# miha-stopar/Plonky3-mobile

Hardware: AMD Instinct MI355X
Metric: fib_air proofs/sec (higher is better)
Workload: dtype u32 (BabyBear Montgomery, 31-bit modular)

## Files before the change

include/p3hip.h:

```cpp
#ifndef P3HIP_H
#define P3HIP_H
#include <stddef.h>
#include <stdint.h>

#ifdef __cplusplus
extern "C" {
#endif

#define P3HIP_OK 0
#define P3HIP_ERR_BAD_ARG (-1)
#define P3HIP_ERR_HIP (-2)
#define P3HIP_ERR_BACKEND (-3)
#define P3HIP_ERR_INTERNAL (-4)

#define P3HIP_BACKEND_CPU 0
#define P3HIP_BACKEND_VULKAN 1
#define P3HIP_BACKEND_METAL 2
#define P3HIP_BACKEND_WEBGPU 3
#define P3HIP_BACKEND_HIP 4

int p3hip_set_backend(const char *name);
int p3hip_get_backend(void);
int p3hip_is_available(char *msg, size_t cap);
const char *p3hip_take_last_error(void);
// ... 10 lines not shown
int p3hip_coset_dft_batch_bb31(const uint32_t *in, uint32_t *out, size_t height, size_t width,
                               uint32_t shift_monty);
int p3hip_coset_lde_batch_bb31(const uint32_t *in, uint32_t *out, size_t height, size_t width,
                               unsigned added_bits, uint32_t shift_monty, int bit_reversed_out);
const char *p3hip_last_timing_line(void);
int p3hip_dft_batch_bb31_dev(const uint32_t *d_in, uint32_t *d_out, size_t height, size_t width, void *stream);
int p3hip_idft_batch_bb31_dev(const uint32_t *d_in, uint32_t *d_out, size_t height, size_t width, void *stream);
int p3hip_coset_dft_batch_bb31_dev(const uint32_t *d_in, uint32_t *d_out, size_t height, size_t width,
                                   uint32_t shift_monty, void *stream);
int p3hip_coset_lde_batch_bb31_dev(const uint32_t *d_in, uint32_t *d_out, size_t height, size_t width,
                                   unsigned added_bits, uint32_t shift_monty, int bit_reversed_out,
                                   void *stream);
int p3hip_coset_lde_from_coeffs_bb31_dev(const uint32_t *d_coeffs, uint32_t *d_out, size_t height, size_t width,
                                         unsigned added_bits, uint32_t shift_monty, void *stream);
int p3hip_dft_plan_bb31(size_t height, size_t width, uint32_t *stages_per_pass, size_t cap, size_t *n_passes);
int p3hip_bit_reverse_rows_dev(const uint32_t *d_in, uint32_t *d_out, size_t height, size_t width, void *stream);

int p3hip_fib_trace_dev(uint64_t a, uint64_t b, size_t n, uint32_t *d_out, void *stream);

int p3hip_poseidon2_permute_dev(uint32_t *d_states, size_t n, void *stream);
int p3hip_poseidon2_permute(uint32_t *states, size_t n);
int p3hip_poseidon2_permute_variant_dev(uint32_t *d_states, size_t n, int variant, void *stream);
int p3hip_poseidon2_f64_probe_dev(const double *d_in, uint32_t *d_out, size_t n, int mode, void *stream);

typedef struct p3hip_tree p3hip_tree_t;
int p3hip_mmcs_commit_dev(const uint32_t *const *d_mats, const size_t *heights, const size_t *widths,
                          size_t n_mats, uint32_t root_out[8], p3hip_tree_t **tree_out, void *stream);
int p3hip_mmcs_commit_async_dev(const uint32_t *const *d_mats, const size_t *heights, const size_t *widths,
                                size_t n_mats, p3hip_tree_t **tree_out, void *stream);
int p3hip_mmcs_root(const p3hip_tree_t *tree, uint32_t root_out[8], void *stream);
size_t p3hip_mmcs_log_max_height(const p3hip_tree_t *tree);
size_t p3hip_mmcs_num_layers(const p3hip_tree_t *tree);
const uint32_t *p3hip_mmcs_layer_dev(const p3hip_tree_t *tree, size_t layer, size_t *len_out);
int p3hip_mmcs_open_batch(const p3hip_tree_t *tree, size_t index, uint32_t *rows_out, uint32_t *path_out,
                          void *stream);
void p3hip_mmcs_free(p3hip_tree_t *tree);
int p3hip_mmcs_commit(const uint32_t *const *mats, const size_t *heights, const size_t *widths,
                      size_t n_mats, uint32_t root_out[8], p3hip_tree_t **tree_out);

#define P3HIP_HASH_POSEIDON2 0
#define P3HIP_HASH_KECCAK 1
int p3hip_mmcs_commit_hash_dev(int hash, const uint32_t *const *d_mats, const size_t *heights, const size_t *widths,
                               size_t n_mats, uint32_t root_out[8], p3hip_tree_t **tree_out, void *stream);
int p3hip_mmcs_commit_hash(int hash, const uint32_t *const *mats, const size_t *heights, const size_t *widths,
                           size_t n_mats, uint32_t root_out[8], p3hip_tree_t **tree_out);
size_t p3hip_mmcs_layer_words(size_t max_height);
// ... 91 lines not shown
```

plonky3-mobile_amd/_lib.py:

```python
import ctypes as C
import os
import subprocess

_HERE = os.path.dirname(os.path.abspath(__file__))
LIB_PATH = os.environ.get("P3HIP_LIB") or os.path.join(_HERE, "libp3hip.so")
ROOT = os.path.dirname(_HERE)

u32p = C.POINTER(C.c_uint32)
_SIGS = {
    "p3hip_set_backend": (C.c_int, [C.c_char_p]),
    "p3hip_get_backend": (C.c_int, []),
    "p3hip_is_available": (C.c_int, [C.c_char_p, C.c_size_t]),
    "p3hip_take_last_error": (C.c_char_p, []),
    "p3hip_malloc": (C.c_int, [C.POINTER(C.c_void_p), C.c_size_t]),
    "p3hip_free": (C.c_int, [C.c_void_p]),
    "p3hip_upload": (C.c_int, [C.c_void_p, C.c_void_p, C.c_size_t]),
    "p3hip_download": (C.c_int, [C.c_void_p, C.c_void_p, C.c_size_t]),
    "p3hip_sync": (C.c_int, [C.c_void_p]),
    "p3hip_last_timing_line": (C.c_char_p, []),
    "p3hip_release_thread_context": (None, []),
    "p3hip_dft_batch_bb31": (C.c_int, [C.c_void_p, C.c_void_p, C.c_size_t, C.c_size_t]),
    "p3hip_idft_batch_bb31": (C.c_int, [C.c_void_p, C.c_void_p, C.c_size_t, C.c_size_t]),
    "p3hip_coset_dft_batch_bb31": (C.c_int, [C.c_void_p, C.c_void_p, C.c_size_t, C.c_size_t, C.c_uint32]),
    "p3hip_coset_lde_batch_bb31": (C.c_int, [C.c_void_p, C.c_void_p, C.c_size_t, C.c_size_t, C.c_uint,
                                             C.c_uint32, C.c_int]),
    "p3hip_dft_batch_bb31_dev": (C.c_int, [C.c_void_p, C.c_void_p, C.c_size_t, C.c_size_t, C.c_void_p]),
    "p3hip_idft_batch_bb31_dev": (C.c_int, [C.c_void_p, C.c_void_p, C.c_size_t, C.c_size_t, C.c_void_p]),
    "p3hip_coset_dft_batch_bb31_dev": (C.c_int, [C.c_void_p, C.c_void_p, C.c_size_t, C.c_size_t, C.c_uint32,
                                                 C.c_void_p]),
    "p3hip_coset_lde_batch_bb31_dev": (C.c_int, [C.c_void_p, C.c_void_p, C.c_size_t, C.c_size_t, C.c_uint,
                                                 C.c_uint32, C.c_int, C.c_void_p]),
    "p3hip_coset_lde_from_coeffs_bb31_dev": (C.c_int, [C.c_void_p, C.c_void_p, C.c_size_t, C.c_size_t, C.c_uint, C.c_uint32,
                                                       C.c_void_p]),
    "p3hip_bit_reverse_rows_dev": (C.c_int, [C.c_void_p, C.c_void_p, C.c_size_t, C.c_size_t, C.c_void_p]),
    "p3hip_dft_plan_bb31": (C.c_int, [C.c_size_t, C.c_size_t, C.POINTER(C.c_uint32), C.c_size_t, C.POINTER(C.c_size_t)]),
    "p3hip_fib_trace_dev": (C.c_int, [C.c_uint64, C.c_uint64, C.c_size_t, C.c_void_p, C.c_void_p]),
    "p3hip_poseidon2_permute_dev": (C.c_int, [C.c_void_p, C.c_size_t, C.c_void_p]),
    "p3hip_poseidon2_permute": (C.c_int, [C.c_void_p, C.c_size_t]),
    "p3hip_poseidon2_permute_variant_dev": (C.c_int, [C.c_void_p, C.c_size_t, C.c_int, C.c_void_p]),
    "p3hip_poseidon2_f64_probe_dev": (C.c_int, [C.c_void_p, C.c_void_p, C.c_size_t, C.c_int, C.c_void_p]),
    "p3hip_mmcs_commit_dev": (C.c_int, [C.POINTER(C.c_void_p), C.POINTER(C.c_size_t), C.POINTER(C.c_size_t),
                                        C.c_size_t, C.c_void_p, C.POINTER(C.c_void_p), C.c_void_p]),
    "p3hip_mmcs_commit_async_dev": (C.c_int, [C.POINTER(C.c_void_p), C.POINTER(C.c_size_t),
                                              C.POINTER(C.c_size_t), C.c_size_t, C.POINTER(C.c_void_p),
                                              C.c_void_p]),
    "p3hip_mmcs_commit_hash_dev": (C.c_int, [C.c_int, C.POINTER(C.c_void_p), C.POINTER(C.c_size_t), C.POINTER(C.c_size_t),
                                             C.c_size_t, C.c_void_p, C.POINTER(C.c_void_p), C.c_void_p]),
    "p3hip_mmcs_commit_hash": (C.c_int, [C.c_int, C.POINTER(C.c_void_p), C.POINTER(C.c_size_t), C.POINTER(C.c_size_t),
                                         C.c_size_t, C.c_void_p, C.POINTER(C.c_void_p)]),
    "p3hip_mmcs_layer_words": (C.c_size_t, [C.c_size_t]),
    "p3hip_mmcs_commit_into_dev": (C.c_int, [C.c_int, C.POINTER(C.c_void_p), C.POINTER(C.c_size_t), C.POINTER(C.c_size_t),
                                             C.c_size_t, C.c_void_p, C.POINTER(C.c_void_p), C.c_void_p]),
    "p3hip_keccak_f_dev": (C.c_int, [C.c_void_p, C.c_size_t, C.c_void_p]),
    "p3hip_mmcs_root": (C.c_int, [C.c_void_p, C.c_void_p, C.c_void_p]),
    "p3hip_mmcs_log_max_height": (C.c_size_t, [C.c_void_p]),
    "p3hip_mmcs_num_layers": (C.c_size_t, [C.c_void_p]),
    "p3hip_mmcs_layer_dev": (C.c_void_p, [C.c_void_p, C.c_size_t, C.POINTER(C.c_size_t)]),
    "p3hip_mmcs_open_batch": (C.c_int, [C.c_void_p, C.c_size_t, C.c_void_p, C.c_void_p, C.c_void_p]),
    "p3hip_mmcs_free": (None, [C.c_void_p]),
    "p3hip_set_thread_profile": (C.c_int, [C.c_int]),
    "p3hip_get_thread_profile": (C.c_int, []),
    "p3hip_fib_prover_create_profile": (C.c_int, [C.c_int, C.c_int, C.c_int, C.c_uint64, C.c_uint, C.c_void_p, C.c_void_p, C.c_int,
                                                  C.POINTER(C.c_void_p)]),
# ... 126 lines not shown
```

plonky3-mobile_amd/csrc/c_api.hip:

```cpp
#include "../../include/p3hip.h"

#include <atomic>
#include <chrono>
#include <condition_variable>
#include <mutex>
#include <deque>
#include <thread>
#include <cctype>
#include <cstdio>
#include <cstring>

#include "bb31.hip.h"
#include "common.h"
#include "mmcs.h"
#include "prover.h"
#include "rng.h"

namespace p3 {
bool take_error(std::string* out);
}
using namespace p3;

static std::atomic<uint8_t> g_backend{P3HIP_BACKEND_HIP};

// ... 269 lines not shown
        P3_HIP(hipMemcpy(states, cx->ws(stream, 2).ptr, n * 64, hipMemcpyDeviceToHost));
        return OK;
    });
}

int p3hip_poseidon2_permute_variant_dev(uint32_t* d_states, size_t n, int variant, void* stream) {
    return guarded([&]() -> int {
        if (n && !d_states) return fail(ERR_BAD_ARG, "null state pointer");
        if (variant != 0 && variant != 1) return fail(ERR_BAD_ARG, "poseidon2 variant: 0 = int32, 1 = fp64");
        Context* cx;
        int rc = get_context(&cx);
        if (rc) return rc;
        return poseidon2_permute_states_variant((hipStream_t)stream, d_states, n, variant);
    });
}
int p3hip_poseidon2_f64_probe_dev(const double* d_in, uint32_t* d_out, size_t n, int mode, void* stream) {
    return guarded([&]() -> int {
        if (n && (!d_in || !d_out)) return fail(ERR_BAD_ARG, "null pointer");
        if (mode < 0 || mode > 2) return fail(ERR_BAD_ARG, "probe mode: 0 = permutation, 1 = internal rounds, 2 = reduce");
        Context* cx;
        int rc = get_context(&cx);
        if (rc) return rc;
        return poseidon2_f64_probe((hipStream_t)stream, d_in, d_out, n, mode);
    });
}

}
struct p3hip_tree {
    Tree* t;
};
extern "C" {

static int commit_async_kind(int kind, const uint32_t* const* d_mats, const size_t* heights, const size_t* widths,
                             size_t n_mats, p3hip_tree_t** tree_out, void* stream) {
    return guarded([&]() -> int {
        if (!tree_out) return fail(ERR_BAD_ARG, "mmcs_commit: null tree_out");
        Context* cx;
        int rc = get_context(&cx);
        if (rc) return rc;
        Tree* t = nullptr;
        rc = mmcs_commit((hipStream_t)stream, d_mats, heights, widths, n_mats, &t, nullptr, nullptr, kind, nullptr, cx->profile);
        if (rc) return rc;
        *tree_out = new p3hip_tree{t};
        return OK;
    });
}
// ... 705 lines not shown
```

plonky3-mobile_amd/csrc/mmcs.h:

```cpp
#pragma once
#include <memory>
#include <cstring>
#include "common.h"

namespace p3 {

enum HashKind : int { HASH_POSEIDON2 = 0, HASH_KECCAK = 1 };

struct Tree {
    int kind = HASH_POSEIDON2;
    std::vector<const uint32_t*> mats;
    std::vector<size_t> heights, widths, strides;
    std::vector<void*> owned;
    uint32_t* layers = nullptr;
    bool root_copied = false;
    bool owns_layers = true;
    std::vector<size_t> layer_off, layer_len;
    uint32_t log_max_height = 0;
    uint32_t* staging = nullptr;
    size_t staging_words = 0;
    ~Tree();
};

int mmcs_commit(hipStream_t stream, const uint32_t* const* d_mats, const size_t* heights, const size_t* widths,
                size_t n_mats, Tree** out, uint32_t* ext_layers = nullptr, uint32_t* root_copy = nullptr,
                int kind = HASH_POSEIDON2, const size_t* strides = nullptr, int profile = PROFILE_LATENCY);
inline size_t mmcs_layer_words(uint64_t max_height) { return (size_t)(2 * max_height - 1) * 8; }
int mmcs_root(hipStream_t stream, const Tree& t, uint32_t root_out[8]);
int mmcs_open(hipStream_t stream, const Tree& t, uint64_t index, uint32_t* rows_out, uint32_t* path_out);
int poseidon2_permute_states(hipStream_t stream, uint32_t* d_states, uint64_t n);
int poseidon2_f64_probe(hipStream_t stream, const double* d_in, uint32_t* d_out, uint64_t n, int mode);
int poseidon2_permute_states_variant(hipStream_t stream, uint32_t* d_states, uint64_t n, int variant);
int keccak_f_states(hipStream_t stream, uint64_t* d_states, uint64_t n);

}
```

plonky3-mobile_amd/csrc/mmcs.hip:

```cpp
#include <algorithm>

#include "common.h"
#include "mmcs.h"
#include "poseidon2.hip.h"
#include "poseidon2_coop.hip.h"
#include "poseidon2_f64.hip.h"
#include "poseidon2_q4.hip.h"
#include "keccak.hip.h"

namespace p3 {

constexpr int MAX_CLASS_MATS = 16;

struct RowSet {
    const uint32_t* ptr[MAX_CLASS_MATS];
    uint32_t width[MAX_CLASS_MATS];
    uint32_t stride[MAX_CLASS_MATS];
    uint32_t count;
    uint32_t total;
};

__device__ __forceinline__ void load_digest(const uint32_t* p, uint32_t* out8) {
    const uint4* q = reinterpret_cast<const uint4*>(p);
    uint4 a = q[0], b = q[1];
// ... 94 lines not shown
    if (gridDim.x <= 512u) P3_LATENCY_BOUND_KERNEL();
    uint64_t r = (uint64_t)blockIdx.x * blockDim.x + threadIdx.x;
    if (r >= n_rows) return;
    double s[16];
#pragma unroll
    for (int i = 0; i < 16; i++) s[i] = 0.0;
    const uint32_t* row = mat + r * width;
    for (uint32_t k = 0; k < width; k += 8) {
#pragma unroll
        for (int i = 0; i < 8; i++)
            if (k + i < width) s[i] = p2f::load_elem(row[k + i]);
        p2f::permute(s);
        if (k + 8 < width) {
#pragma unroll
            for (int i = 0; i < 16; i++) s[i] = p2f::reduce(s[i]);
        }
    }
    uint32_t d[8];
    const p2f::MagicRegs smk = p2f::magic_regs();
#pragma unroll
    for (int i = 0; i < 8; i++) d[i] = p2f::store_elem(s[i], smk);
    store_digest(digests + r * 8, d);
}
__global__ void __launch_bounds__(256) compress_layer_q4_kernel(const uint32_t* prev, uint32_t* next, uint64_t n_out, uint32_t prio) {
    if (prio) P3_LATENCY_BOUND_KERNEL();
    const uint32_t q = threadIdx.x & 3u;
    const uint64_t i = ((uint64_t)blockIdx.x * blockDim.x + threadIdx.x) >> 2;
    const bool act = i < n_out;
    const p2q::LaneConsts lc = p2q::lane_consts(q);
    double s[4] = {0.0, 0.0, 0.0, 0.0};
    if (act) {
        const uint4 w = *reinterpret_cast<const uint4*>(prev + i * 16 + 4 * q);
        s[0] = p2f::load_elem(w.x); s[1] = p2f::load_elem(w.y); s[2] = p2f::load_elem(w.z); s[3] = p2f::load_elem(w.w);
    }
    p2q::permute(s, lc, q == 0);
    if (act && q < 2) {
        const p2f::MagicRegs smk = p2f::magic_regs();
        *reinterpret_cast<uint4*>(next + i * 8 + 4 * q) =
            make_uint4(p2f::store_elem(s[0], smk), p2f::store_elem(s[1], smk), p2f::store_elem(s[2], smk), p2f::store_elem(s[3], smk));
    }
}
__global__ void __launch_bounds__(256) leaf_hash_q4_kernel(const uint32_t* mat, uint32_t width, uint64_t n_rows, uint32_t* digests, uint32_t prio) {
    if (prio) P3_LATENCY_BOUND_KERNEL();
    const uint32_t q = threadIdx.x & 3u;
    const uint64_t r = ((uint64_t)blockIdx.x * blockDim.x + threadIdx.x) >> 2;
    const bool act = r < n_rows;
// ... 56 lines not shown
            }
        }
    }
    if (r >= n_rows) return;
    uint32_t d[8];
    const p2f::MagicRegs smk = p2f::magic_regs();
#pragma unroll
    for (int i = 0; i < 8; i++) d[i] = p2f::store_elem(s[i], smk);
    store_digest(digests + r * 8, d);
}
__global__ void __launch_bounds__(256) leaf_hash_f64_rowset_kernel(RowSet rs, uint64_t n_rows, uint32_t* digests) {
    if (gridDim.x <= 512u) P3_LATENCY_BOUND_KERNEL();
    uint64_t r = (uint64_t)blockIdx.x * blockDim.x + threadIdx.x;
    if (r >= n_rows) return;
    double s[16];
#pragma unroll
    for (int i = 0; i < 16; i++) s[i] = 0.0;
    uint32_t m = 0, off = 0;
    for (uint32_t k = 0; k < rs.total; k += 8) {
#pragma unroll
        for (int i = 0; i < 8; i++) {
            if (k + i < rs.total) {
                while (off >= rs.width[m]) { m++; off = 0; }
                s[i] = p2f::load_elem(rs.ptr[m][r * rs.stride[m] + off]);
                off++;
            }
        }
        p2f::permute(s);
        if (k + 8 < rs.total) {
#pragma unroll
            for (int i = 0; i < 16; i++) s[i] = p2f::reduce(s[i]);
        }
    }
    uint32_t d[8];
    const p2f::MagicRegs smk = p2f::magic_regs();
#pragma unroll
    for (int i = 0; i < 8; i++) d[i] = p2f::store_elem(s[i], smk);
    store_digest(digests + r * 8, d);
}
__global__ void __launch_bounds__(256) compress_layer_f64_kernel(const uint32_t* prev, uint32_t* next, uint64_t n_out) {
    if (gridDim.x <= 512u) P3_LATENCY_BOUND_KERNEL();
    uint64_t i = (uint64_t)blockIdx.x * blockDim.x + threadIdx.x;
    if (i >= n_out) return;
    uint32_t w[16];
    load_digest(prev + i * 16, w);
    load_digest(prev + i * 16 + 8, w + 8);
    double s[16];
#pragma unroll
    for (int k = 0; k < 16; k++) s[k] = p2f::load_elem(w[k]);
    p2f::permute(s);
    uint32_t d[8];
    const p2f::MagicRegs smk = p2f::magic_regs();
#pragma unroll
    for (int k = 0; k < 8; k++) d[k] = p2f::store_elem(s[k], smk);
    store_digest(next + i * 8, d);
}

__global__ void __launch_bounds__(256) compress_coop_kernel(const uint32_t* prev, uint32_t* next, uint32_t n_out) {
    P3_LATENCY_BOUND_KERNEL();
    const uint32_t lane16 = threadIdx.x & 15;
    const p2c::LaneConst lc = p2c::lane_constants(lane16);
    uint32_t i = (blockIdx.x * blockDim.x + threadIdx.x) >> 4;
    bool act = i < n_out;
    uint32_t v = act ? prev[(size_t)i * 16 + lane16] : 0u;
    v = p2c::permute(v, lc);
    if (act && lane16 < 8) next[(size_t)i * 8 + lane16] = v;
}
__global__ void __launch_bounds__(256) leaf_coop_kernel(const uint32_t* mat, uint32_t width, uint32_t n_rows, uint32_t* digests) {
    P3_LATENCY_BOUND_KERNEL();
    const uint32_t lane16 = threadIdx.x & 15;
    const p2c::LaneConst lc = p2c::lane_constants(lane16);
    uint32_t r = (blockIdx.x * blockDim.x + threadIdx.x) >> 4;
    bool act = r < n_rows;
// ... 62 lines not shown
#pragma unroll
    for (int k = 0; k < 4; k++)
        q[k] = make_uint4(p2f::store_elem(s[4 * k]), p2f::store_elem(s[4 * k + 1]), p2f::store_elem(s[4 * k + 2]), p2f::store_elem(s[4 * k + 3]));
}

__global__ void poseidon2_f64_probe_kernel(const double* in, uint32_t* out, uint64_t n, int mode) {
    uint64_t i = (uint64_t)blockIdx.x * blockDim.x + threadIdx.x;
    if (i >= n) return;
    double s[16];
#pragma unroll
    for (int k = 0; k < 16; k++) s[k] = in[i * 16 + k];
    if (mode == 0) p2f::permute(s);
    else if (mode == 1) p2f::internal_rounds(s, p2f::magic_regs());
    else {
#pragma unroll
        for (int k = 0; k < 16; k++) s[k] = p2f::reduce(s[k]);
    }
#pragma unroll
    for (int k = 0; k < 16; k++) out[i * 16 + k] = p2f::store_elem(s[k]);
}
int poseidon2_f64_probe(hipStream_t stream, const double* d_in, uint32_t* d_out, uint64_t n, int mode) {
    if (!n) return OK;
    hipLaunchKernelGGL(poseidon2_f64_probe_kernel, dim3((uint32_t)((n + 255) / 256)), dim3(256), 0, stream, d_in, d_out, n, mode);
    P3_HIP(hipGetLastError());
    return OK;
}
int poseidon2_permute_states_variant(hipStream_t stream, uint32_t* d_states, uint64_t n, int variant) {
    if (!n) return OK;
    if (variant == 1) hipLaunchKernelGGL(poseidon2_permute_f64_kernel, dim3((uint32_t)((n + 255) / 256)), dim3(256), 0, stream, d_states, n);
    else hipLaunchKernelGGL(poseidon2_permute_kernel, dim3((uint32_t)((n + 255) / 256)), dim3(256), 0, stream, d_states, n);
    P3_HIP(hipGetLastError());
    return OK;
}

int poseidon2_permute_states(hipStream_t stream, uint32_t* d_states, uint64_t n) {
    return poseidon2_permute_states_variant(stream, d_states, n, 1);
}

__device__ __forceinline__ uint32_t rowset_elem(const RowSet& rs, uint64_t r, uint32_t k, uint32_t& m, uint32_t& base) {
    while (k - base >= rs.width[m]) { base += rs.width[m]; m++; }
    return rs.ptr[m][r * rs.stride[m] + (k - base)];
}
__device__ __forceinline__ void keccak_sponge_row(const RowSet& rs, uint64_t r, uint64_t (&st)[25]) {
#pragma unroll
    for (int i = 0; i < 25; i++) st[i] = 0;
    const uint32_t n = rs.total, n64 = (n + 1) / 2;
// ... 367 lines not shown
                if (t->layer_len[l + levels - 1] == 1) t->root_copied = root_copy != nullptr;
                l += levels - 1;
                continue;
            }
            hipLaunchKernelGGL(keccak_compress_kernel, dim3((uint32_t)((len + 255) / 256)), dim3(256), 0, stream,
                               t->layers + t->layer_off[l - 1], t->layers + t->layer_off[l], len, rs, rs.count > 0 ? 1u : 0u);
            P3_HIP(hipGetLastError());
        }
        *out = t.release();
        return OK;
    }
    {
        RowSet rs = make_rowset(*t, maxh);
        const bool dense1 = rs.count == 1 && rs.stride[0] == rs.width[0];
        if (dense1 && maxh < COOP_MAX && maxh * 16 <= 0x7fffffffull) {
            hipLaunchKernelGGL(leaf_coop_kernel, dim3((uint32_t)((maxh * 16 + 255) / 256)), dim3(256), 0, stream, rs.ptr[0],
                               rs.width[0], (uint32_t)maxh, t->layers);
        } else if (dense1 && maxh <= Q4_MAX && rs.width[0] <= 64 && (reinterpret_cast<uintptr_t>(t->layers) & 15u) == 0) {
            hipLaunchKernelGGL(leaf_hash_q4_kernel, dim3((uint32_t)((maxh * 4 + 255) / 256)), dim3(256), 0, stream, rs.ptr[0], rs.width[0], maxh,
                               t->layers, Q4_PRIO);
        } else if (dense1 && rs.width[0] >= 64) {
            hipLaunchKernelGGL(leaf_hash_f64_wide_kernel, dim3((uint32_t)((maxh + 255) / 256)), dim3(256), 0, stream, rs.ptr[0],
                               rs.width[0], maxh, t->layers);
        } else if (dense1) {
            hipLaunchKernelGGL(leaf_hash_f64_kernel, dim3((uint32_t)((maxh + 255) / 256)), dim3(256), 0, stream, rs.ptr[0],
                               rs.width[0], maxh, t->layers);
        } else if ((maxh >= COOP_MAX || (rs.count == 1 && !dense1))) {
            hipLaunchKernelGGL(leaf_hash_f64_rowset_kernel, dim3((uint32_t)((maxh + 255) / 256)), dim3(256), 0, stream, rs, maxh, t->layers);
        } else {
            hipLaunchKernelGGL(leaf_hash_kernel, dim3((uint32_t)((maxh + 255) / 256)), dim3(256), 0, stream, rs, maxh, t->layers);
        }
        P3_HIP(hipGetLastError());
    }
    for (size_t l = 1; l < t->layer_len.size();) {
        uint64_t len = t->layer_len[l];
        RowSet rs = make_rowset(*t, len);
        bool inject = rs.count > 0;
        if (!inject && len < COOP_MAX) {
            uint32_t levels = 0;
            while (levels < COOP_CHUNK_LOG && l + levels < t->layer_len.size() && !has_height(*t, t->layer_len[l + levels])) levels++;
            uint64_t n_in = t->layer_len[l - 1];
            uint32_t chunk = (uint32_t)std::min<uint64_t>(n_in, 1ull << COOP_CHUNK_LOG);
            while ((1u << levels) > chunk) levels--;
            uint32_t blocks = (uint32_t)(n_in / chunk);
            uint32_t threads = std::max<uint32_t>(64, chunk * 8);
            bool makes_root = t->layer_len[l + levels - 1] == 1;
// ... 59 lines not shown
```

plonky3-mobile_amd/csrc/poseidon2_f64.hip.h:

```cpp
#pragma once
#include "poseidon2.hip.h"

namespace p2f {

constexpr double PD = 2013265921.0;
constexpr double PINV = 1.0 / 2013265921.0;

__device__ __forceinline__ double mulmod(double a, double b) {
    double h = a * b;
    double l = __fma_rn(a, b, -h);
    double q = __builtin_rint(h * PINV);
    double r = __fma_rn(-q, PD, h);
    return r + l;
}
constexpr double PM1 = 2013265920.0;
__device__ __forceinline__ double mulmod_p(double a, double b, double aP) {
    double q = __builtin_rint(b * aP);
    double t = __fma_rn(a, b, -(q * PM1));
    return t - q;
}
__device__ __forceinline__ double reduce(double x) {
    return __fma_rn(-__builtin_rint(x * PINV), PD, x);
}
__device__ __forceinline__ double add_scaled_pow2(double tot, double x, double inv) {
// ... 84 lines not shown
        s[8] = __fma_rn(s[8], -4.0, tot);
        s[9] = add_scaled_pow2(tot, s[9], i256);
        s[10] = add_scaled_pow2(tot, s[10], i4);
        s[11] = add_scaled_pow2(tot, s[11], i8);
        s[12] = __fma_rn(s[12], -k15, tot);
        s[13] = add_scaled_pow2(tot, s[13], -i256);
        s[14] = add_scaled_pow2(tot, s[14], -i16);
        s[15] = __fma_rn(s[15], k15, tot);
    };
    auto fold_integer_lanes = [&]() {
        s[1] = reduce(s[1]); s[2] = reduce(s[2]); s[4] = reduce(s[4]); s[5] = reduce(s[5]);
        s[7] = reduce(s[7]); s[8] = reduce(s[8]); s[12] = reduce(s[12]); s[15] = reduce(s[15]);
    };
    _Pragma("clang loop unroll(disable)")
    for (int blk = 0; blk < 3; blk++) {
        _Pragma("clang loop unroll(disable)")
        for (int r = 0; r < 4; r++) internal_round(4 * blk + r);
        fold_integer_lanes();
    }
    internal_round(12);
    fold_integer_lanes();
}

__device__ __forceinline__ void permute(double (&s)[16]) {
    const MagicRegs mk = magic_regs();
    const double npm1 = d_c.neg_pm1, pinv = d_c.pinv;
    external_linear(s);
    _Pragma("clang loop unroll(disable)")
    for (int r = 0; r < 4; r++) {
#pragma unroll
        for (int i = 0; i < 16; i++) s[i] = sbox7(s[i] + d_c.ext[r][i], mk, npm1, pinv);
        external_linear(s);
    }
    internal_rounds(s, mk);
    _Pragma("clang loop unroll(disable)")
    for (int r = 4; r < 8; r++) {
#pragma unroll
        for (int i = 0; i < 16; i++) s[i] = sbox7(s[i] + d_c.ext[r][i], mk, npm1, pinv);
        external_linear(s);
    }
}

__device__ __forceinline__ double load_elem(uint32_t monty) { return (double)bb::from_monty(monty); }
constexpr double R_MOD_P = 268435454.0;
constexpr double R_MOD_P_OVER_P = 268435454.0 / 2013265921.0;
__device__ __forceinline__ uint32_t store_elem(double v, const MagicRegs& k) {
    const double r = mulmod_m(R_MOD_P, v, R_MOD_P_OVER_P, k, d_c.neg_pm1);
    const uint32_t w = (uint32_t)(int32_t)r;
    return min(w, w + bb::P);
}
__device__ __forceinline__ uint32_t store_elem(double v) { return store_elem(v, magic_regs()); }

}
```

plonky3-mobile_amd/csrc/prover.hip:

```cpp
#include <chrono>
#include <deque>
#include <memory>
#include <cstring>

#include "bb31.hip.h"
#include "challenger.h"
#include "common.h"
#include "keccak.hip.h"
#include "mmcs.h"
#include "poseidon2.hip.h"
#include "poseidon2_f64.hip.h"
#include "prover.h"
#include "rng.h"
#include "rng_dev.hip.h"
#include "transcript.hip.h"

namespace p3 {

using bb::Ext;

__device__ __forceinline__ uint32_t tl(const TwoLevelTable& t, uint32_t e) {
    return bb::mul(t.lo[e & ((1u << t.T) - 1u)], t.hi[e >> t.T]);
}
__device__ __forceinline__ uint32_t brev(uint32_t v, uint32_t bits) { return bits ? (__brev(v) >> (32 - bits)) : 0u; }
// ... 43 lines not shown
};
__global__ void __launch_bounds__(256) fib_quotient_kernel(QuotArgs a) {
    uint32_t i = blockIdx.x * blockDim.x + threadIdx.x;
    if (i >= a.n) return;
    const DevState* __restrict__ ds = a.ds;
    uint2 loc = a.lde[brev(i, a.log_n)];
    uint2 nxt = a.lde[brev((i + 1) & (a.n - 1), a.log_n)];
    uint2 s = a.sel[i];
    uint32_t x = bb::mul(a.gen, tl(a.roots, i));
    uint32_t trans = bb::sub(x, a.ginv);
    uint32_t c0 = bb::mul(s.x, bb::sub(loc.x, ds->pis[0]));
    uint32_t c1 = bb::mul(s.x, bb::sub(loc.y, ds->pis[1]));
    uint32_t c2 = bb::mul(trans, bb::sub(loc.y, nxt.x));
    uint32_t c3 = bb::mul(trans, bb::sub(bb::add(loc.x, loc.y), nxt.y));
    uint32_t c4 = bb::mul(s.y, bb::sub(loc.y, ds->pis[2]));
    Ext acc;
#pragma unroll
    for (int k = 0; k < 4; k++)
        acc.c[k] = bb::add(bb::add(bb::dot2(ds->apow[4].c[k], c0, ds->apow[3].c[k], c1), bb::dot2(ds->apow[2].c[k], c2, ds->apow[1].c[k], c3)),
                           bb::mul(ds->apow[0].c[k], c4));
    st_ext(a.out + 4 * (size_t)i, bb::scale(acc, a.zh_inv));
}

constexpr int DEN_CHUNK = 4;
__global__ void __launch_bounds__(256) inv_denoms_kernel(TwoLevelTable roots, uint32_t big, uint32_t log_big, uint32_t gen,
                                                         const DevState* __restrict__ ds, uint32_t* d0, uint32_t* d1) {
    const DenConsts k0 = ds->k0, k1 = ds->k1;
    uint32_t t = blockIdx.x * blockDim.x + threadIdx.x;
    uint32_t j0 = t * DEN_CHUNK;
    if (j0 >= big) return;
    uint32_t a0[2 * DEN_CHUNK], e0[2 * DEN_CHUNK], e1[2 * DEN_CHUNK], nrm[2 * DEN_CHUNK], pre[2 * DEN_CHUNK];
#pragma unroll
    for (int k = 0; k < DEN_CHUNK; k++) {
        uint32_t x = bb::mul(gen, tl(roots, brev((j0 + k) & (big - 1), log_big)));
#pragma unroll
        for (int z = 0; z < 2; z++) {
            const DenConsts& c = z ? k1 : k0;
            const uint32_t a = bb::sub(c.z0, x);
            const uint32_t dd0 = bb::add(bb::sqr(a), c.k0), dd1 = bb::sub(bb::mul(c.k1, a), c.c1);
            a0[2 * k + z] = a; e0[2 * k + z] = dd0; e1[2 * k + z] = dd1;
            nrm[2 * k + z] = bb::sub(bb::sqr(dd0), bb::mul(bb::W_MONTY, bb::sqr(dd1)));
        }
    }
    uint32_t acc = bb::ONE;
#pragma unroll
    for (int k = 0; k < 2 * DEN_CHUNK; k++) { pre[k] = acc; acc = bb::mul(acc, nrm[k]); }
    uint32_t inv = bb::inv(acc);
// ... 93 lines not shown
                         bb::mul(ds->alp[1].c[c], t.y));
        w.c[c] = bb::dot2(ds->alp[2].c[c], t.x, ds->alp[3].c[c], t.y);
    }
    u.c[0] = bb::add(u.c[0], t.x);
    Ext e0 = ld_ext(a.d0 + 4 * (size_t)j), e1 = ld_ext(a.d1 + 4 * (size_t)j);
    Ext r = bb::add(bb::mul(bb::sub(ds->y02, u), e0), bb::mul(bb::sub(ds->y1, w), e1));
    st_ext(a.ro + 4 * (size_t)j, r);
}

__global__ void __launch_bounds__(256) fri_fold_kernel(TwoLevelTable inv_roots , const uint32_t* in,
                                                       uint32_t* out, uint32_t half, uint32_t log_half,
                                                       const DevState* __restrict__ ds, uint32_t round, uint32_t one_half) {
    if (gridDim.x <= 512u) P3_LATENCY_BOUND_KERNEL();
    uint32_t i = blockIdx.x * blockDim.x + threadIdx.x;
    if (i >= half) return;
    const Ext half_beta = ds->half_beta[round];
    Ext lo = ld_ext(in + 8 * (size_t)i), hi = ld_ext(in + 8 * (size_t)i + 4);
    uint32_t p = tl(inv_roots, brev(i, log_half));
    Ext s = bb::scale(bb::add(lo, hi), one_half);
    Ext d = bb::mul(bb::scale(half_beta, p), bb::sub(lo, hi));
    st_ext(out + 4 * (size_t)i, bb::add(s, d));
}

__global__ void __launch_bounds__(256) grind_kernel(DevState* ds, uint32_t mask, uint32_t base) {
    uint32_t w = base + blockIdx.x * blockDim.x + threadIdx.x;
    if (w >= bb::P) return;
    if (base + blockIdx.x * blockDim.x > *(volatile uint32_t*)&ds->grind_result) return;
    const uint32_t pos = ds->n_in;
    double s[16];
#pragma unroll
    for (int i = 0; i < 16; i++) s[i] = p2f::load_elem((i < 8 && (uint32_t)i < pos) ? ds->inb[i & 7] : ds->st[i]);
#pragma unroll
    for (int i = 0; i < 8; i++) s[i] = (i == (int)pos) ? (double)w : s[i];
    p2f::permute(s);
    if ((bb::from_monty(p2f::store_elem(s[7])) & mask) == 0) atomicMin(&ds->grind_result, w);
}

__global__ void __launch_bounds__(256) grind_keccak_kernel(DevState* ds, uint32_t mask, uint32_t base) {
    uint32_t w = base + blockIdx.x * blockDim.x + threadIdx.x;
    if (w >= bb::P) return;
    if (base + blockIdx.x * blockDim.x > *(volatile uint32_t*)&ds->grind_result) return;
    const KeccakGrindArgs& a = ds->kgrind;
    const uint32_t wm = bb::to_monty(w);
    uint64_t st[25];
#pragma unroll
    for (int i = 0; i < 25; i++) st[i] = a.state[i];
    for (uint32_t blk = 0; blk < a.n_blocks; blk++) {
#pragma unroll
        for (int i = 0; i < 17; i++) {
            uint64_t lane = a.block[blk][i];
            const int32_t rel = (int32_t)(a.wpos) - (int32_t)(blk * 136 + i * 8);
            if (rel > -4 && rel < 8) {
                const uint64_t v = (uint64_t)wm;
                lane ^= rel >= 0 ? (v << (8 * rel)) : (v >> (8 * -rel));
            }
            st[i] ^= lane;
        }
        if (blk + 1 == a.n_blocks) kk::permute_digest(st);
        else kk::permute(st);
    }
    bool ok = false;
#pragma unroll
    for (int t = 0; t < 8; t++) {
        const uint64_t lane = st[3 - t / 2];
        const uint32_t hi_or_lo = (t & 1) ? (uint32_t)lane : (uint32_t)(lane >> 32);
        const uint32_t v = __builtin_bswap32(hi_or_lo) & 0x7fffffffu;
        if (v < bb::P) { ok = (v & mask) == 0; break; }
    }
    if (ok) atomicMin(&ds->grind_result, w);
}

constexpr uint32_t QTREE_MAX_MATS = 8;
struct QTree {
    const uint32_t* mat[QTREE_MAX_MATS];
    uint32_t width[QTREE_MAX_MATS];
    uint32_t stride[QTREE_MAX_MATS];
    uint32_t n_mats;
    const uint32_t* layers;
    uint32_t log_height, shift, slot_off;
};
__global__ void query_gather_kernel(const QTree* trees, const uint32_t* indices, uint32_t slot_words, uint32_t* out) {
    P3_LATENCY_BOUND_KERNEL();
    const QTree& t = trees[blockIdx.y];
    const uint64_t index = (indices[blockIdx.x] >> t.shift) & ((1ull << t.log_height) - 1ull);
    uint32_t* dst = out + (size_t)blockIdx.x * slot_words + t.slot_off;
    uint32_t off = 0;
    for (uint32_t m = 0; m < t.n_mats; m++) {
        for (uint32_t c = threadIdx.x; c < t.width[m]; c += blockDim.x) dst[off + c] = t.mat[m][index * t.stride[m] + c];
        off += t.width[m];
    }
    uint64_t base = 0, len = 1ull << t.log_height;
    for (uint32_t i = 0; i < t.log_height; i++) {
// ... 408 lines not shown
            P3_HIP(hipGetLastError());
            TwoLevelTable inv_roots;
            if ((rc = cx.get_root_table(stream, log_half + 1, true, &inv_roots))) return rc;
            hipLaunchKernelGGL(fri_fold_kernel, dim3((half + 255) / 256), dim3(256), 0, stream, inv_roots, vec, fri_vec + fri_vec_off[r + 1],
                               half, log_half, ts.ds, r, one_half);
            P3_HIP(hipGetLastError());
        }
        return OK;
    }
    int fri_final(Context& cx, const TsArgs& ts) {
        const uint32_t fpl = 1u << fp.log_final_poly_len;
        int rc;
        if ((rc = bit_reverse_rows(stream, fri_vec + fri_vec_off[n_rounds], fp_ev, fpl, 4))) return rc;
        if ((rc = ntt_dft(cx, stream, fp_ev, pstage + lay.fpoly, fpl, 4, true))) return rc;
        hipLaunchKernelGGL(ts_final_kernel, dim3(1), dim3(64), 0, stream, ts, fpl, pow_mask());
        P3_HIP(hipGetLastError());
        return OK;
    }

    uint32_t pow_mask() const { return (1u << fp.proof_of_work_bits) - 1u; }
    uint32_t grind_range(uint32_t first_log) const {
        return 1u << std::min<uint32_t>(std::max<uint32_t>(first_log ? first_log : fp.proof_of_work_bits + 4, 8), 24);
    }
    int grind(const TsArgs& ts, uint64_t base, uint32_t count) {
        if (hash == HASH_KECCAK) hipLaunchKernelGGL(grind_keccak_kernel, dim3(count / 256), dim3(256), 0, stream, ts.ds, pow_mask(), (uint32_t)base);
        else hipLaunchKernelGGL(grind_kernel, dim3(count / 256), dim3(256), 0, stream, ts.ds, pow_mask(), (uint32_t)base);
        P3_HIP(hipGetLastError());
        return OK;
    }
    int grind_start(const TsArgs& ts) {
        const uint32_t first_log = grind_first_log(), batch = grind_range(first_log);
        const uint32_t head = first_log ? batch : std::min<uint32_t>(batch, 1u << std::max<uint32_t>(fp.proof_of_work_bits + 1, 8));
        int rc;
        if ((rc = grind(ts, 0, head))) return rc;
        if (batch > head && (rc = grind(ts, head, batch - head))) return rc;
        return OK;
    }
    int queries(const TsArgs& ts, uint32_t* host, size_t words) {
        const uint32_t nq = fp.num_queries;
        hipLaunchKernelGGL(ts_queries_kernel, dim3(1), dim3(64), 0, stream, ts, nq, log_big, fp.proof_of_work_bits, qidx);
        P3_HIP(hipGetLastError());
        if (nq) {
            hipLaunchKernelGGL(query_gather_kernel, dim3(nq, (uint32_t)trees.size()), dim3(64), 0, stream, qtrees, qidx, (uint32_t)slot_words,
                               pstage + lay.slots);
            P3_HIP(hipGetLastError());
        }
        P3_HIP(hipMemcpyAsync(host, pstage, words * 4, hipMemcpyDeviceToHost, stream));
        return OK;
    }
    int continue_grind(const TsArgs& ts, uint32_t* host, size_t words) {
        uint32_t batch = grind_range(grind_first_log()), found = 0xffffffffu;
        int rc;
        for (uint64_t base = batch; base < bb::P && found == 0xffffffffu; base += batch) {
            batch = std::min<uint32_t>(batch * 4, 1u << 24);
            if ((rc = grind(ts, base, batch))) return rc;
            P3_HIP(hipMemcpyAsync(&found, &ts.ds->grind_result, 4, hipMemcpyDeviceToHost, stream));
            P3_HIP(hipStreamSynchronize(stream));
        }
        if (found == 0xffffffffu) return fail(ERR_INTERNAL, "grind: no proof-of-work witness found");
        if ((rc = queries(ts, host, words))) return rc;
        P3_HIP(hipStreamSynchronize(stream));
        return OK;
    }

    void put_fri(std::vector<uint8_t>& pf, const uint32_t* hp) const {
        const StageLayout& L = lay;
        const uint32_t nq = fp.num_queries, fpl = 1u << fp.log_final_poly_len, n_inputs = (uint32_t)trees.size() - n_rounds;
        put_u32(pf, n_rounds); put_words(pf, hp + L.froots, (size_t)n_rounds * 8);
        put_u32(pf, nq);
        for (uint32_t q = 0; q < nq; q++) {
            const uint32_t* slot = hp + L.slots + (size_t)q * slot_words;
            put_u32(pf, n_inputs);
            for (uint32_t i = 0; i < n_inputs; i++) {
                const QTree& t = trees[i];
                put_opening(pf, slot, salt_words ? t.n_mats / 2 : t.n_mats, t.width, salt_words, t.log_height);
            }
            put_u32(pf, n_rounds);
            for (uint32_t r = 0; r < n_rounds; r++) {
// ... 315 lines not shown
```

Measured before the change: 507.9.

## Use negated-element Poseidon2 path, width-specialized leaf hashing, and persistent grind kernels

```diff
diff --git a/include/p3hip.h b/include/p3hip.h
--- a/include/p3hip.h
+++ b/include/p3hip.h
@@ -56,6 +56,7 @@
 int p3hip_poseidon2_permute(uint32_t *states, size_t n);
 int p3hip_poseidon2_permute_variant_dev(uint32_t *d_states, size_t n, int variant, void *stream);
 int p3hip_poseidon2_f64_probe_dev(const double *d_in, uint32_t *d_out, size_t n, int mode, void *stream);
+int p3hip_poseidon2_compress_layer_dev(const uint32_t *d_prev, uint32_t *d_next, size_t n_out, void *stream);
 
 typedef struct p3hip_tree p3hip_tree_t;
 int p3hip_mmcs_commit_dev(const uint32_t *const *d_mats, const size_t *heights, const size_t *widths,
diff --git a/plonky3-mobile_amd/_lib.py b/plonky3-mobile_amd/_lib.py
--- a/plonky3-mobile_amd/_lib.py
+++ b/plonky3-mobile_amd/_lib.py
@@ -39,6 +39,7 @@
     "p3hip_poseidon2_permute": (C.c_int, [C.c_void_p, C.c_size_t]),
     "p3hip_poseidon2_permute_variant_dev": (C.c_int, [C.c_void_p, C.c_size_t, C.c_int, C.c_void_p]),
     "p3hip_poseidon2_f64_probe_dev": (C.c_int, [C.c_void_p, C.c_void_p, C.c_size_t, C.c_int, C.c_void_p]),
+    "p3hip_poseidon2_compress_layer_dev": (C.c_int, [C.c_void_p, C.c_void_p, C.c_size_t, C.c_void_p]),
     "p3hip_mmcs_commit_dev": (C.c_int, [C.POINTER(C.c_void_p), C.POINTER(C.c_size_t), C.POINTER(C.c_size_t),
                                         C.c_size_t, C.c_void_p, C.POINTER(C.c_void_p), C.c_void_p]),
     "p3hip_mmcs_commit_async_dev": (C.c_int, [C.POINTER(C.c_void_p), C.POINTER(C.c_size_t),
diff --git a/plonky3-mobile_amd/csrc/c_api.hip b/plonky3-mobile_amd/csrc/c_api.hip
--- a/plonky3-mobile_amd/csrc/c_api.hip
+++ b/plonky3-mobile_amd/csrc/c_api.hip
@@ -315,6 +315,17 @@
         int rc = get_context(&cx);
         if (rc) return rc;
         return poseidon2_f64_probe((hipStream_t)stream, d_in, d_out, n, mode);
+    });
+}
+int p3hip_poseidon2_compress_layer_dev(const uint32_t* d_prev, uint32_t* d_next, size_t n_out, void* stream) {
+    return guarded([&]() -> int {
+        if (n_out && (!d_prev || !d_next)) return fail(ERR_BAD_ARG, "null pointer");
+        if ((reinterpret_cast<uintptr_t>(d_prev) | reinterpret_cast<uintptr_t>(d_next)) & 15u) return fail(ERR_BAD_ARG, "compress_layer: digests must be 16-byte aligned");
+        if (n_out > (1ull << 31)) return fail(ERR_BAD_ARG, "compress_layer: more than 2^31 digests");
+        Context* cx;
+        int rc = get_context(&cx);
+        if (rc) return rc;
+        return poseidon2_compress_layer((hipStream_t)stream, d_prev, d_next, n_out);
     });
 }
 
diff --git a/plonky3-mobile_amd/csrc/mmcs.h b/plonky3-mobile_amd/csrc/mmcs.h
--- a/plonky3-mobile_amd/csrc/mmcs.h
+++ b/plonky3-mobile_amd/csrc/mmcs.h
@@ -30,6 +30,7 @@
 int mmcs_open(hipStream_t stream, const Tree& t, uint64_t index, uint32_t* rows_out, uint32_t* path_out);
 int poseidon2_permute_states(hipStream_t stream, uint32_t* d_states, uint64_t n);
 int poseidon2_f64_probe(hipStream_t stream, const double* d_in, uint32_t* d_out, uint64_t n, int mode);
+int poseidon2_compress_layer(hipStream_t stream, const uint32_t* d_prev, uint32_t* d_next, uint64_t n_out);
 int poseidon2_permute_states_variant(hipStream_t stream, uint32_t* d_states, uint64_t n, int variant);
 int keccak_f_states(hipStream_t stream, uint64_t* d_states, uint64_t n);
 
diff --git a/plonky3-mobile_amd/csrc/mmcs.hip b/plonky3-mobile_amd/csrc/mmcs.hip
--- a/plonky3-mobile_amd/csrc/mmcs.hip
+++ b/plonky3-mobile_amd/csrc/mmcs.hip
@@ -140,6 +140,32 @@
     for (int i = 0; i < 8; i++) d[i] = p2f::store_elem(s[i], smk);
     store_digest(digests + r * 8, d);
 }
+template <int W>
+__global__ void __launch_bounds__(256) leaf_hash_f64_w_kernel(const uint32_t* __restrict__ mat, uint64_t n_rows, uint32_t* __restrict__ digests) {
+    if (gridDim.x <= 512u) P3_LATENCY_BOUND_KERNEL();
+    const uint64_t r = (uint64_t)blockIdx.x * blockDim.x + threadIdx.x;
+    if (r >= n_rows) return;
+    uint32_t w[W];
+    if constexpr (W == 2) {
+        const uint2 v = reinterpret_cast<const uint2*>(mat)[r];
+        w[0] = v.x; w[1] = v.y;
+    } else {
+#pragma unroll
+        for (int k = 0; k < W; k += 4) {
+            const uint4 v = reinterpret_cast<const uint4*>(mat)[r * (W / 4) + k / 4];
+            w[k] = v.x; w[k + 1] = v.y; w[k + 2] = v.z; w[k + 3] = v.w;
+        }
+    }
+    double u[W], s[16];
+#pragma unroll
+    for (int k = 0; k < W; k++) u[k] = p2f::load_elem_neg(w[k]);
+    p2f::permute_neg_first_block<W>(u, s);
+    uint32_t d[8];
+    const p2f::MagicRegs smk = p2f::magic_regs();
+#pragma unroll
+    for (int i = 0; i < 8; i++) d[i] = p2f::store_elem(s[i], smk);
+    store_digest(digests + r * 8, d);
+}
 __global__ void __launch_bounds__(256) compress_layer_q4_kernel(const uint32_t* prev, uint32_t* next, uint64_t n_out, uint32_t prio) {
     if (prio) P3_LATENCY_BOUND_KERNEL();
     const uint32_t q = threadIdx.x & 3u;
@@ -242,14 +268,14 @@
         for (int i = 0; i < 8; i++) {
             if (k + i < rs.total) {
                 while (off >= rs.width[m]) { m++; off = 0; }
-                s[i] = p2f::load_elem(rs.ptr[m][r * rs.stride[m] + off]);
+                s[i] = p2f::load_elem_neg(rs.ptr[m][r * rs.stride[m] + off]);
                 off++;
             }
         }
-        p2f::permute(s);
+        p2f::permute_neg(s);
         if (k + 8 < rs.total) {
 #pragma unroll
-            for (int i = 0; i < 16; i++) s[i] = p2f::reduce(s[i]);
+            for (int i = 0; i < 16; i++) s[i] = p2f::reduce_neg(s[i]);
         }
     }
     uint32_t d[8];
@@ -267,8 +293,8 @@
     load_digest(prev + i * 16 + 8, w + 8);
     double s[16];
 #pragma unroll
-    for (int k = 0; k < 16; k++) s[k] = p2f::load_elem(w[k]);
-    p2f::permute(s);
+    for (int k = 0; k < 16; k++) s[k] = p2f::load_elem_neg(w[k]);
+    p2f::permute_neg(s);
     uint32_t d[8];
     const p2f::MagicRegs smk = p2f::magic_regs();
 #pragma unroll
@@ -377,6 +403,12 @@
 int poseidon2_f64_probe(hipStream_t stream, const double* d_in, uint32_t* d_out, uint64_t n, int mode) {
     if (!n) return OK;
     hipLaunchKernelGGL(poseidon2_f64_probe_kernel, dim3((uint32_t)((n + 255) / 256)), dim3(256), 0, stream, d_in, d_out, n, mode);
+    P3_HIP(hipGetLastError());
+    return OK;
+}
+int poseidon2_compress_layer(hipStream_t stream, const uint32_t* d_prev, uint32_t* d_next, uint64_t n_out) {
+    if (!n_out) return OK;
+    hipLaunchKernelGGL(compress_layer_f64_kernel, dim3((uint32_t)((n_out + 255) / 256)), dim3(256), 0, stream, d_prev, d_next, n_out);
     P3_HIP(hipGetLastError());
     return OK;
 }
@@ -790,6 +822,12 @@
         } else if (dense1 && rs.width[0] >= 64) {
             hipLaunchKernelGGL(leaf_hash_f64_wide_kernel, dim3((uint32_t)((maxh + 255) / 256)), dim3(256), 0, stream, rs.ptr[0],
                                rs.width[0], maxh, t->layers);
+        } else if (dense1 && (rs.width[0] == 2 || rs.width[0] == 4 || rs.width[0] == 8) &&
+                   (reinterpret_cast<uintptr_t>(rs.ptr[0]) & (rs.width[0] == 2 ? 7u : 15u)) == 0) {
+            const dim3 grid((uint32_t)((maxh + 255) / 256));
+            if (rs.width[0] == 2) hipLaunchKernelGGL(leaf_hash_f64_w_kernel<2>, grid, dim3(256), 0, stream, rs.ptr[0], maxh, t->layers);
+            else if (rs.width[0] == 4) hipLaunchKernelGGL(leaf_hash_f64_w_kernel<4>, grid, dim3(256), 0, stream, rs.ptr[0], maxh, t->layers);
+            else hipLaunchKernelGGL(leaf_hash_f64_w_kernel<8>, grid, dim3(256), 0, stream, rs.ptr[0], maxh, t->layers);
         } else if (dense1) {
             hipLaunchKernelGGL(leaf_hash_f64_kernel, dim3((uint32_t)((maxh + 255) / 256)), dim3(256), 0, stream, rs.ptr[0],
                                rs.width[0], maxh, t->layers);
diff --git a/plonky3-mobile_amd/csrc/poseidon2_f64.hip.h b/plonky3-mobile_amd/csrc/poseidon2_f64.hip.h
--- a/plonky3-mobile_amd/csrc/poseidon2_f64.hip.h
+++ b/plonky3-mobile_amd/csrc/poseidon2_f64.hip.h
@@ -130,10 +130,9 @@
     fold_integer_lanes();
 }
 
-__device__ __forceinline__ void permute(double (&s)[16]) {
+__device__ __forceinline__ void permute_rounds(double (&s)[16]) {
     const MagicRegs mk = magic_regs();
     const double npm1 = d_c.neg_pm1, pinv = d_c.pinv;
-    external_linear(s);
     _Pragma("clang loop unroll(disable)")
     for (int r = 0; r < 4; r++) {
 #pragma unroll
@@ -147,6 +146,54 @@
         for (int i = 0; i < 16; i++) s[i] = sbox7(s[i] + d_c.ext[r][i], mk, npm1, pinv);
         external_linear(s);
     }
+}
+__device__ __forceinline__ void permute(double (&s)[16]) {
+    external_linear(s);
+    permute_rounds(s);
+}
+
+__device__ __forceinline__ double load_elem_neg(uint32_t monty) { return (double)__umulhi(monty * bb::MU, bb::P); }
+__device__ __forceinline__ void mat4_neg(double& a, double& b, double& c, double& d) {
+    double t01 = -a - b, t23 = -c - d, t0123 = t01 + t23;
+    double t01123 = t0123 - b, t01233 = t0123 - d;
+    double nd = __fma_rn(a, -2.0, t01233), nb = __fma_rn(c, -2.0, t01123);
+    double na = t01123 + t01, nc = t01233 + t23;
+    a = na; b = nb; c = nc; d = nd;
+}
+__device__ __forceinline__ void permute_neg(double (&s)[16]) {
+#pragma unroll
+    for (int i = 0; i < 16; i += 4) mat4_neg(s[i], s[i + 1], s[i + 2], s[i + 3]);
+    double t[4];
+#pragma unroll
+    for (int k = 0; k < 4; k++) t[k] = (s[k] + s[k + 4]) + (s[k + 8] + s[k + 12]);
+#pragma unroll
+    for (int i = 0; i < 16; i++) s[i] += t[i & 3];
+    permute_rounds(s);
+}
+__device__ __forceinline__ double reduce_neg(double x) { return __fma_rn(__builtin_rint(x * PINV), PD, -x); }
+template <int W>
+__device__ __forceinline__ void permute_neg_first_block(const double (&u)[W], double (&s)[16]) {
+    static_assert(W == 2 || W == 4 || W == 8, "one sponge block of 2, 4 or 8 words");
+    double a[8];
+    if constexpr (W == 2) {
+        const double t01 = -u[0] - u[1], t011 = t01 - u[1];
+        a[0] = t011 + t01; a[1] = t011; a[2] = t01; a[3] = __fma_rn(u[0], -2.0, t01);
+    } else {
+#pragma unroll
+        for (int i = 0; i < W; i++) a[i] = u[i];
+#pragma unroll
+        for (int i = 0; i < W; i += 4) mat4_neg(a[i], a[i + 1], a[i + 2], a[i + 3]);
+    }
+#pragma unroll
+    for (int k = 0; k < 4; k++) {
+        if constexpr (W == 8) {
+            const double t = a[k] + a[k + 4];
+            s[k] = a[k] + t; s[k + 4] = a[k + 4] + t; s[k + 8] = t; s[k + 12] = t;
+        } else {
+            s[k] = a[k] + a[k]; s[k + 4] = a[k]; s[k + 8] = a[k]; s[k + 12] = a[k];
+        }
+    }
+    permute_rounds(s);
 }
 
 __device__ __forceinline__ double load_elem(uint32_t monty) { return (double)bb::from_monty(monty); }
diff --git a/plonky3-mobile_amd/csrc/prover.hip b/plonky3-mobile_amd/csrc/prover.hip
--- a/plonky3-mobile_amd/csrc/prover.hip
+++ b/plonky3-mobile_amd/csrc/prover.hip
@@ -89,7 +89,7 @@
     st_ext(a.out + 4 * (size_t)i, bb::scale(acc, a.zh_inv));
 }
 
-constexpr int DEN_CHUNK = 4;
+constexpr int DEN_CHUNK = 8;
 __global__ void __launch_bounds__(256) inv_denoms_kernel(TwoLevelTable roots, uint32_t big, uint32_t log_big, uint32_t gen,
                                                          const DevState* __restrict__ ds, uint32_t* d0, uint32_t* d1) {
     const DenConsts k0 = ds->k0, k1 = ds->k1;
@@ -229,52 +229,61 @@
     st_ext(out + 4 * (size_t)i, bb::add(s, d));
 }
 
-__global__ void __launch_bounds__(256) grind_kernel(DevState* ds, uint32_t mask, uint32_t base) {
-    uint32_t w = base + blockIdx.x * blockDim.x + threadIdx.x;
-    if (w >= bb::P) return;
-    if (base + blockIdx.x * blockDim.x > *(volatile uint32_t*)&ds->grind_result) return;
+__global__ void __launch_bounds__(256) grind_kernel(DevState* ds, uint32_t mask, uint32_t base, uint32_t count) {
     const uint32_t pos = ds->n_in;
-    double s[16];
-#pragma unroll
-    for (int i = 0; i < 16; i++) s[i] = p2f::load_elem((i < 8 && (uint32_t)i < pos) ? ds->inb[i & 7] : ds->st[i]);
-#pragma unroll
-    for (int i = 0; i < 8; i++) s[i] = (i == (int)pos) ? (double)w : s[i];
-    p2f::permute(s);
-    if ((bb::from_monty(p2f::store_elem(s[7])) & mask) == 0) atomicMin(&ds->grind_result, w);
-}
-
-__global__ void __launch_bounds__(256) grind_keccak_kernel(DevState* ds, uint32_t mask, uint32_t base) {
-    uint32_t w = base + blockIdx.x * blockDim.x + threadIdx.x;
-    if (w >= bb::P) return;
-    if (base + blockIdx.x * blockDim.x > *(volatile uint32_t*)&ds->grind_result) return;
-    const KeccakGrindArgs& a = ds->kgrind;
-    const uint32_t wm = bb::to_monty(w);
-    uint64_t st[25];
-#pragma unroll
-    for (int i = 0; i < 25; i++) st[i] = a.state[i];
-    for (uint32_t blk = 0; blk < a.n_blocks; blk++) {
-#pragma unroll
-        for (int i = 0; i < 17; i++) {
-            uint64_t lane = a.block[blk][i];
-            const int32_t rel = (int32_t)(a.wpos) - (int32_t)(blk * 136 + i * 8);
-            if (rel > -4 && rel < 8) {
-                const uint64_t v = (uint64_t)wm;
-                lane ^= rel >= 0 ? (v << (8 * rel)) : (v >> (8 * -rel));
+    uint32_t m[16];
+#pragma unroll
+    for (int i = 0; i < 16; i++) m[i] = (i < 8 && (uint32_t)i < pos) ? ds->inb[i & 7] : ds->st[i];
+    for (uint32_t blk = blockIdx.x; blk < count / 256u; blk += gridDim.x) {
+        const uint32_t start = base + blk * 256u;
+        if (start > *(volatile uint32_t*)&ds->grind_result) return;
+        const uint32_t w = start + threadIdx.x;
+        if (w >= bb::P) return;
+        double s[16];
+#pragma unroll
+        for (int i = 0; i < 16; i++) s[i] = p2f::load_elem_neg(m[i]);
+#pragma unroll
+        for (int i = 0; i < 8; i++) s[i] = (i == (int)pos) ? (double)(bb::P - w) : s[i];
+        p2f::permute_neg(s);
+        if ((bb::from_monty(p2f::store_elem(s[7])) & mask) == 0) atomicMin(&ds->grind_result, w);
+    }
+}
+
+__global__ void __launch_bounds__(256) grind_keccak_kernel(DevState* ds, uint32_t mask, uint32_t base, uint32_t count) {
+    for (uint32_t cblk = blockIdx.x; cblk < count / 256u; cblk += gridDim.x) {
+        const uint32_t start = base + cblk * 256u;
+        if (start > *(volatile uint32_t*)&ds->grind_result) return;
+        const uint32_t w = start + threadIdx.x;
+        if (w >= bb::P) return;
+        const KeccakGrindArgs& a = ds->kgrind;
+        const uint32_t wm = bb::to_monty(w);
+        uint64_t st[25];
+#pragma unroll
+        for (int i = 0; i < 25; i++) st[i] = a.state[i];
+        for (uint32_t blk = 0; blk < a.n_blocks; blk++) {
+#pragma unroll
+            for (int i = 0; i < 17; i++) {
+                uint64_t lane = a.block[blk][i];
+                const int32_t rel = (int32_t)(a.wpos) - (int32_t)(blk * 136 + i * 8);
+                if (rel > -4 && rel < 8) {
+                    const uint64_t v = (uint64_t)wm;
+                    lane ^= rel >= 0 ? (v << (8 * rel)) : (v >> (8 * -rel));
+                }
+                st[i] ^= lane;
             }
-            st[i] ^= lane;
-        }
-        if (blk + 1 == a.n_blocks) kk::permute_digest(st);
-        else kk::permute(st);
-    }
-    bool ok = false;
-#pragma unroll
-    for (int t = 0; t < 8; t++) {
-        const uint64_t lane = st[3 - t / 2];
-        const uint32_t hi_or_lo = (t & 1) ? (uint32_t)lane : (uint32_t)(lane >> 32);
-        const uint32_t v = __builtin_bswap32(hi_or_lo) & 0x7fffffffu;
-        if (v < bb::P) { ok = (v & mask) == 0; break; }
-    }
-    if (ok) atomicMin(&ds->grind_result, w);
+            if (blk + 1 == a.n_blocks) kk::permute_digest(st);
+            else kk::permute(st);
+        }
+        bool ok = false;
+#pragma unroll
+        for (int t = 0; t < 8; t++) {
+            const uint64_t lane = st[3 - t / 2];
+            const uint32_t hi_or_lo = (t & 1) ? (uint32_t)lane : (uint32_t)(lane >> 32);
+            const uint32_t v = __builtin_bswap32(hi_or_lo) & 0x7fffffffu;
+            if (v < bb::P) { ok = (v & mask) == 0; break; }
+        }
+        if (ok) atomicMin(&ds->grind_result, w);
+    }
 }
 
 constexpr uint32_t QTREE_MAX_MATS = 8;
@@ -729,18 +738,21 @@
     uint32_t grind_range(uint32_t first_log) const {
         return 1u << std::min<uint32_t>(std::max<uint32_t>(first_log ? first_log : fp.proof_of_work_bits + 4, 8), 24);
     }
-    int grind(const TsArgs& ts, uint64_t base, uint32_t count) {
-        if (hash == HASH_KECCAK) hipLaunchKernelGGL(grind_keccak_kernel, dim3(count / 256), dim3(256), 0, stream, ts.ds, pow_mask(), (uint32_t)base);
-        else hipLaunchKernelGGL(grind_kernel, dim3(count / 256), dim3(256), 0, stream, ts.ds, pow_mask(), (uint32_t)base);
+    int grind(const TsArgs& ts, uint64_t base, uint32_t count, uint32_t grid) {
+        grid = std::max<uint32_t>(1, std::min<uint32_t>(grid, count / 256));
+        if (hash == HASH_KECCAK) hipLaunchKernelGGL(grind_keccak_kernel, dim3(grid), dim3(256), 0, stream, ts.ds, pow_mask(), (uint32_t)base, count);
+        else hipLaunchKernelGGL(grind_kernel, dim3(grid), dim3(256), 0, stream, ts.ds, pow_mask(), (uint32_t)base, count);
         P3_HIP(hipGetLastError());
         return OK;
     }
+    static constexpr uint32_t GRIND_GRID = 64;
     int grind_start(const TsArgs& ts) {
         const uint32_t first_log = grind_first_log(), batch = grind_range(first_log);
+        if (profile != PROFILE_LATENCY) return grind(ts, 0, batch, GRIND_GRID);
         const uint32_t head = first_log ? batch : std::min<uint32_t>(batch, 1u << std::max<uint32_t>(fp.proof_of_work_bits + 1, 8));
         int rc;
-        if ((rc = grind(ts, 0, head))) return rc;
-        if (batch > head && (rc = grind(ts, head, batch - head))) return rc;
+        if ((rc = grind(ts, 0, head, head / 256))) return rc;
+        if (batch > head && (rc = grind(ts, head, batch - head, (batch - head) / 256))) return rc;
         return OK;
     }
     int queries(const TsArgs& ts, uint32_t* host, size_t words) {
@@ -760,7 +772,7 @@
         int rc;
         for (uint64_t base = batch; base < bb::P && found == 0xffffffffu; base += batch) {
             batch = std::min<uint32_t>(batch * 4, 1u << 24);
-            if ((rc = grind(ts, base, batch))) return rc;
+            if ((rc = grind(ts, base, batch, profile != PROFILE_LATENCY ? 16 * GRIND_GRID : batch / 256))) return rc;
             P3_HIP(hipMemcpyAsync(&found, &ts.ds->grind_result, 4, hipMemcpyDeviceToHost, stream));
             P3_HIP(hipStreamSynchronize(stream));
         }
```

Result: no change. 502.3 (median of 2 runs) (-1.1%).
